# wuxiyang1996/iPLAN

Hardware: AMD Instinct MI355X
Metric: env-steps/sec (whole node), Hetero-Highway chaotic 5-agent (higher is better)
Workload: dtype f32; 1 GPU; Highway chaotic full iPLAN (Behaviour + GAT + soft update), 5 agents x 55 entities, 32 envs/GPU x 90 steps; step = 8 rollouts, each followed by insert + Behavior_policy.learn + Prediction_policy.learn, then IPPOLearner.train (15 epochs x 255 x 90 rows x 5 agents); envs_per_gpu=32

## Files before the change

include/iplan_hip.h:

```cpp
#ifndef IPLAN_HIP_H
#define IPLAN_HIP_H

#include <stddef.h>
#include <stdint.h>

#ifdef __cplusplus
extern "C" {
#endif

typedef void* iplan_stream_t;

enum {
    IPLAN_OK = 0,
    IPLAN_EINVAL = -1,
    IPLAN_EALIGN = -2,
    IPLAN_EHIP = -3
};

const char* iplan_last_error(void);
int iplan_version(void);
size_t iplan_sizeof(const char* struct_name);

#define IPLAN_MAX_ENTITIES 64
#define IPLAN_GAT_HIDDEN 32
// ... 347 lines not shown
    float clip, huber_delta, value_loss_coef;
    float* g_logp;
    float* g_values;
    float* stats;
    const float* mask_sum;
    int32_t flags;
    float row_count;
    int32_t n_parts;
} IplanPpoLossArgs;
#define IPLAN_PPO_MSE 1
#define IPLAN_PPO_NO_VCLIP 2
#define IPLAN_PPO_VALUE_MEAN 4
#define IPLAN_PPO_POLICY_MEAN 8

int iplan_ppo_loss(const IplanPpoLossArgs* args, iplan_stream_t stream);

#define IPLAN_GAT_NODE_DY 640
#define IPLAN_GAT_HARD_PART (8 * IPLAN_GAT_HIDDEN + 16)
#define IPLAN_GAT_WHH_PART (3 * IPLAN_GAT_HIDDEN * IPLAN_GAT_HIDDEN + 3 * IPLAN_GAT_HIDDEN)

typedef struct {
    IplanGatFwdArgs fwd;
    const float* g_out;
    int64_t g_s_net, g_s_b;
    float* dgru;
    float* node_dy;
    float* hard_part;
    float* whh_part;
    float* grad;
    int64_t grad_s_net;
// ... 227 lines not shown
```

iplan_amd/_lib.py:

```python
import ctypes as C
import os

import torch

_HERE = os.path.dirname(os.path.abspath(__file__))
LIB_PATH = os.environ.get("IPLAN_HIP_LIB", os.path.join(_HERE, "libiplan_hip.so"))

GAT_NPARAM = 20
GAT_PARAM_ORDER = [
    "encoding.weight", "encoding.bias",
    "hard_bi_GRU.weight_ih_l0", "hard_bi_GRU.weight_hh_l0", "hard_bi_GRU.bias_ih_l0", "hard_bi_GRU.bias_hh_l0",
    "hard_bi_GRU.weight_ih_l0_reverse", "hard_bi_GRU.weight_hh_l0_reverse",
    "hard_bi_GRU.bias_ih_l0_reverse", "hard_bi_GRU.bias_hh_l0_reverse",
    "hard_encoding.weight", "hard_encoding.bias",
    "q.weight", "k.weight", "v.weight", "v.bias",
    "rnn.weight_ih", "rnn.weight_hh", "rnn.bias_ih", "rnn.bias_hh",
]

fp = C.c_void_p
i32 = C.c_int32
i64 = C.c_int64


class GatSaved(C.Structure):
# ... 8 lines not shown
        ("h_prev", fp), ("h_s_net", i64), ("h_s_b", i64),
        ("out", fp), ("out_s_net", i64), ("out_s_b", i64),
        ("noise", fp), ("params", fp), ("params_s_net", i64),
        ("off", i64 * GAT_NPARAM), ("tau", C.c_float), ("saved", GatSaved), ("phase_clocks", fp),
    ]


class IplanError(RuntimeError):
    pass


ENTRY_POINTS = ["iplan_gat_fwd", "iplan_enc_fwd", "iplan_ac_fwd", "iplan_adam_step", "iplan_wgrad",
                "iplan_ac_bwd_tail", "iplan_ac_bwd_fc1", "iplan_ac_bwd_fc1_finalize", "iplan_ppo_prepare", "iplan_ppo_adv_norm", "iplan_ppo_loss", "iplan_gat_bwd",
                "iplan_pdec_fwd", "iplan_pdec_bwd", "iplan_beh_fwd", "iplan_beh_bwd", "iplan_mlp3_fwd", "iplan_mlp3_bwd", "iplan_seq2seq_fwd", "iplan_ac_pack_fc1",
                "iplan_ac_xhat_pack", "iplan_ac_fc1_split_fwd", "iplan_ac_bwd_fc1_split",
                "iplan_p2p_publish", "iplan_p2p_reduce", "iplan_obs_history_step", "iplan_seq2seq_bwd", "iplan_predict", "iplan_beh_eval"]
RAW_ENTRY_POINTS = ["iplan_grad_sqnorm", "iplan_wgrad_workspace_floats", "iplan_ac_kpad", "iplan_ac_fc1_groups", "iplan_sizeof", "iplan_ac_packed_floats",
                    "iplan_p2p_alloc", "iplan_p2p_free", "iplan_p2p_export", "iplan_p2p_open", "iplan_p2p_close", "iplan_gat_enc_fwd", "iplan_gat_enc_ac_fwd", "iplan_gumbel_noise", "iplan_ac_xhat_floats", "iplan_ac_fc1_split_chunks", "iplan_ac_fc1_split_parts"]


class Lib:

    def __init__(self, cdll):
        self.c = cdll
        cdll.iplan_last_error.restype = C.c_char_p
        cdll.iplan_version.restype = C.c_int
        for name in ENTRY_POINTS:
            if not hasattr(cdll, name):
                raise IplanError(f"{name} missing from the loaded library")
            fn = getattr(cdll, name)
            fn.restype = C.c_int
            fn.argtypes = [C.c_void_p, C.c_void_p]
        for name in RAW_ENTRY_POINTS:
# ... 215 lines not shown

class PpoLossArgs(C.Structure):
    _fields_ = [
        ("n_agents", i32), ("rows", i32), ("row_stride", i64),
        ("logp", fp), ("entropy", fp), ("values", fp), ("old_logp", fp), ("adv", fp),
        ("value_preds", fp), ("returns", fp), ("mask", fp),
        ("clip", C.c_float), ("huber_delta", C.c_float), ("value_loss_coef", C.c_float),
        ("g_logp", fp), ("g_values", fp), ("stats", fp), ("mask_sum", fp), ("flags", i32), ("row_count", C.c_float),
        ("n_parts", i32),
    ]


PPO_MSE, PPO_NO_VCLIP, PPO_VALUE_MEAN, PPO_POLICY_MEAN = 1, 2, 4, 8


GAT_NODE_DY = 640
GAT_HARD_PART = 8 * 32 + 16
GAT_REC_GROUPS = 8
GAT_WHH_PART = 3 * 32 * 32 + 3 * 32


class GatBwdArgs(C.Structure):
    _fields_ = [("fwd", GatFwdArgs), ("g_out", fp), ("g_s_net", i64), ("g_s_b", i64),
                ("dgru", fp), ("node_dy", fp), ("hard_part", fp), ("whh_part", fp), ("grad", fp), ("grad_s_net", i64)]


DEC_PARAM_ORDER = ["decoder.linear.weight", "decoder.linear.bias", "decoder.rnn.weight_ih_l0", "decoder.rnn.weight_hh_l0",
                   "decoder.rnn.bias_ih_l0", "decoder.rnn.bias_hh_l0", "decoder.out.weight", "decoder.out.bias"]
PDEC_SAVE, PDEC_DSAVE = 256, 176

# ... 75 lines not shown
    _fields_ = [("fwd", Seq2SeqArgs), ("g_out", fp), ("dsave", fp)]


class ObsHistArgs(C.Structure):
    _fields_ = [("K", i32), ("nA", i32), ("N", i32), ("L", i32), ("d", i32), ("obs_num", i32),
                ("obs", fp), ("agent_ids", C.c_void_p), ("slot_id", C.c_void_p), ("n_slots", C.c_void_p), ("win", fp), ("single", fp),
                ("single_s_k", i64), ("single_s_a", i64), ("err", C.c_void_p)]


STRUCT_MIRRORS = {"IplanGatSaved": GatSaved, "IplanGatFwdArgs": GatFwdArgs, "IplanGatBwdArgs": GatBwdArgs,
                  "IplanEncFwdArgs": EncFwdArgs, "IplanAcNet": AcNet, "IplanAcFeatures": AcFeatures, "IplanAcFwdArgs": AcFwdArgs,
                  "IplanAcBwdArgs": AcBwdArgs, "IplanAdamArgs": AdamArgs, "IplanWgradProblem": WgradProblem,
                  "IplanWgradArgs": WgradArgs, "IplanPpoPrepareArgs": PpoPrepareArgs, "IplanPpoLossArgs": PpoLossArgs,
                  "IplanPdecArgs": PdecArgs, "IplanBehArgs": BehArgs, "IplanMlp3Args": Mlp3Args, "IplanAdvNormArgs": AdvNormArgs, "IplanSeq2SeqArgs": Seq2SeqArgs, "IplanSeq2SeqBwdArgs": Seq2SeqBwdArgs, "IplanAcPackArgs": AcPackArgs,
                  "IplanIpcHandle": IpcHandle, "IplanP2pArgs": P2pArgs, "IplanAcXhatArgs": AcXhatArgs, "IplanAcFc1SplitArgs": AcFc1SplitArgs,
                  "IplanObsHistArgs": ObsHistArgs, "IplanPredictArgs": PredictArgs, "IplanBehEvalArgs": BehEvalArgs}
```

iplan_amd/csrc/api.cpp:

```cpp
#include <cstring>

#include "api_util.h"

namespace iplan {
char* error_buffer() {
    static thread_local char buf[512] = {0};
    return buf;
}
}

extern "C" const char* iplan_last_error(void) { return iplan::error_buffer(); }
extern "C" int iplan_version(void) { return 100; }

extern "C" size_t iplan_sizeof(const char* name) {
    if (!name) return 0;
#define IPLAN_SZ(T) if (!strcmp(name, #T)) return sizeof(T);
    IPLAN_SZ(IplanGatSaved) IPLAN_SZ(IplanGatFwdArgs) IPLAN_SZ(IplanGatBwdArgs) IPLAN_SZ(IplanEncFwdArgs) IPLAN_SZ(IplanAcNet)
    IPLAN_SZ(IplanAcFeatures) IPLAN_SZ(IplanAcFwdArgs) IPLAN_SZ(IplanAcBwdArgs) IPLAN_SZ(IplanAdamArgs) IPLAN_SZ(IplanWgradProblem)
    IPLAN_SZ(IplanWgradArgs) IPLAN_SZ(IplanPpoPrepareArgs) IPLAN_SZ(IplanPpoLossArgs) IPLAN_SZ(IplanPdecArgs) IPLAN_SZ(IplanBehArgs) IPLAN_SZ(IplanMlp3Args) IPLAN_SZ(IplanAdvNormArgs) IPLAN_SZ(IplanSeq2SeqArgs) IPLAN_SZ(IplanAcPackArgs) IPLAN_SZ(IplanP2pArgs) IPLAN_SZ(IplanIpcHandle) IPLAN_SZ(IplanAcXhatArgs) IPLAN_SZ(IplanAcFc1SplitArgs) IPLAN_SZ(IplanObsHistArgs) IPLAN_SZ(IplanSeq2SeqBwdArgs)
    IPLAN_SZ(IplanPredictArgs) IPLAN_SZ(IplanBehEvalArgs)
#undef IPLAN_SZ
    return 0;
}
```

iplan_amd/learners/ippo_learner.py:

```python
import copy

import os

import torch as th

from .. import _lib as L
from .. import ops
from ..optim import FusedAdam, step_all
from ..streams import AsyncHost
from ..utils.mappo_utils.util import update_linear_schedule

_STORE_KEYS = ("history", "attention_latent", "behavior_latent", "actions", "avail_actions", "reward",
               "terminated", "rnn_states_actors", "rnn_states_critics", "actions_onehot", "obs", "state")


class EpisodeStore:

    def __init__(self, args, device):
        self.size = args.buffer_size
        self.device = device
        self.count = 0
        self.data = {}
        self.consumed = set()

# ... 265 lines not shown
        stats = th.zeros(self.ppo_epoch, nA, parts, 8, **f32)
        norms = th.zeros(self.ppo_epoch, 2, nA, **f32)
        pl.g_logp, pl.g_values = g_logp.data_ptr(), g_v.data_ptr()
        pl.flags = self._loss_flags
        pl.n_parts = parts
        max_norm = self.max_grad_norm if self._use_max_grad_norm else None
        n_rows = float(rows)
        msum = mask[:, :rows].sum(dim=1).contiguous() if (parts > 1 or self.dp is not None) else None
        if self.dp is not None:
            msum = self.dp.all_reduce_sum(msum)
            n_rows = float(self.dp_global_rows if self.dp_global_rows is not None else rows * self.dp.world)
            pl.row_count = n_rows
        if msum is not None:
            pl.mask_sum = msum.data_ptr()
        xhat = ops.ac_xhat_pack(spec, rows, nA, ln_stats) if split else None
        for ep in range(self.ppo_epoch):
            out = ops.ac_forward(mac.actor_arena, mac.critic_arena, 2, spec, rows, nA, save=True, want_entropy=True, xhat=xhat,
                                 packed=None if xhat is not None else mac.fc1_pack.get(spec), **fwd_kw)
            if split and ep == 0:
                old_logp[:, :rows].copy_(out["logp"])
            pl.logp, pl.entropy, pl.values = out["logp"].data_ptr(), out["entropy"].data_ptr(), out["values"].data_ptr()
            pl.stats = stats[ep].data_ptr()
            lib.call("iplan_ppo_loss", pl, stream)
            ops.ac_backward(out, mac.actor_arena, mac.critic_arena, g_logp=g_logp,
                            g_entropy=-self.entropy_coef / n_rows, g_values=g_v)
            if self.dp is not None:
                self.dp.all_reduce_grads(mac.actor_arena, mac.critic_arena)
            self._probe_before(ep, self.ppo_epoch, out)
            sq_a = step_all(self.actor_optimizers, max_norm)
            norms[ep, 0] = sq_a[:, 0]
            sq_c = step_all(self.critic_optimizers, max_norm)
            norms[ep, 1] = sq_c[:, 0]
            self._probe_after(ep)
        self.store.clear()

        st_d = stats.sum(dim=2).mean(dim=(0, 1))
        nr_d = norms.sqrt().mean(dim=(0, 2)) if max_norm is not None else th.zeros(2, device=dev)

        staged = AsyncHost(th.cat([st_d.reshape(-1), nr_d.reshape(-1)])) if defer else None

# ... 300 lines not shown
```

iplan_amd/ops.py:

```python
import contextlib
import ctypes as C

import os

import torch

from . import _lib as L


def _lib(lib):
    return lib if lib is not None else L.get_lib()


def _nb_strides(t, inner):
    assert t.dtype == torch.float32, t.dtype
    expect = 1
    for d in range(t.dim() - 1, 1, -1):
        assert t.stride(d) == expect or t.shape[d] == 1, (t.shape, t.stride())
        expect *= t.shape[d]
    assert expect == inner, (expect, inner)
    return t.stride(0), t.stride(1)


def _gat_flops(n_nets, B, N, D, A, H=32):
# ... 160 lines not shown
        f.T, f.T_phys = self.T, self.T_phys


def _fill_acnet(dst, arena, order, n_out):
    dst.params = arena.data.data_ptr()
    dst.params_s_net = arena.net_stride
    for i, k in enumerate(order):
        dst.off[i] = arena.off(k)
    dst.n_out = n_out


def ac_forward(actor_arena, critic_arena, which, spec, rows, n_agents, h_actor=None, h_critic=None,
               h_strides=(0, 0), avail=None, avail_strides=(0, 0), mode=0, q_noise=None, actions_in=None,
               act_strides=(0, 0), n_actions=5, ksplit=None, save=False, want_probs=False, want_entropy=False,
               want_h=True, h_out=None, actions_out=None, onehot_out=None, ln_stats=None, ln_stats_mode=0, phase_clocks=None,
               packed=None, xhat=None, lib=None, launch=True):
    lib = _lib(lib)
    dev = (actor_arena if which != 1 else critic_arena).data.device
    a = L.AcFwdArgs()
    a.n_agents, a.rows, a.which = n_agents, rows, which
    a.ksplit = ksplit if ksplit is not None else (8 if rows <= 512 else 1)
    a.act_tanh = int(bool(getattr(actor_arena if which != 1 else critic_arena, "act_tanh", False)))
    if which == 2:
        assert bool(getattr(actor_arena, "act_tanh", False)) == bool(getattr(critic_arena, "act_tanh", False)), \
            "actor and critic of one fused launch must use the same trunk activation (args.use_ReLU)"
    spec.fill(a.feat)
    out = {}
    f32 = dict(dtype=torch.float32, device=dev)
    if which != 1:
        _fill_acnet(a.actor, actor_arena, L.ACTOR_PARAM_ORDER, n_actions)
        a.h_actor = h_actor.data_ptr()
# ... 78 lines not shown
        assert which == 2 and a.ksplit == 1 and ln_stats_mode == 2 and xhat["rows"] == rows and xhat["n_agents"] == n_agents
        s = L.AcFc1SplitArgs()
        s.n_agents, s.rows = n_agents, rows
        spec.fill(s.feat)
        s.actor, s.critic = a.actor, a.critic
        KS = (xhat["KT"] + 1) // 2
        ws = workspace(dev, n_agents * KS * 6144 + 2 * n_agents * L.AC_HIDDEN, "fc1_split")
        kparts = int(lib.c.iplan_ac_fc1_split_parts(n_agents, rows))
        z1 = torch.empty(kparts, 2, n_agents, rows, L.AC_HIDDEN, **f32)
        s.kparts, a.fc1_pre_parts = kparts, kparts
        s.xf, s.wsplit, s.wbeta, s.z1 = xhat["xf"].data_ptr(), ws.data_ptr(), ws.data_ptr() + 4 * n_agents * KS * 6144, z1.data_ptr()
        _launch("ac_fc1_split_fwd", lambda: lib.call("iplan_ac_fc1_split_fwd", s, L.current_stream(dev)),
                work=2.0 * n_agents * rows * spec.F * 2 * L.AC_HIDDEN)
        a.fc1_pre = z1.data_ptr()
        out["_xhat"] = xhat
    if launch:
        _launch("ac_fwd_kernel:train" if save else ("ac_fwd_kernel:rollout" if rows <= 512 else "ac_fwd_kernel:infer"),
                lambda: lib.call("iplan_ac_fwd", a, L.current_stream(dev)))
    else:
        assert a.ksplit == 8 and not save and xhat is None and a.ln_stats_mode == 0, "launch=False is for the rollout-shaped forward"
    out["_args"] = a
    out["_keep"] = (spec, h_actor, h_critic, avail, q_noise, actions_in, h_out, actions_out, onehot_out, ln_stats, packed, z1, xhat, ks_bufs)
    return out


def ac_xhat_pack(spec, rows, n_agents, ln_stats, lib=None):
    lib = _lib(lib)
    dev = ln_stats.device
    a = L.AcXhatArgs()
    a.n_agents, a.rows = n_agents, rows
    spec.fill(a.feat)
# ... 230 lines not shown
    w.add(dptr + 4 * M, dst, M, rows, 1, x=sptr + 4 * M, x_strides=sst, K=M,
          dw_off=off("base.mlp.fc2.0.0.weight"), db_off=off("base.mlp.fc2.0.0.bias"))
    w.add(dptr, dst, M, rows, 1, db_off=off("base.mlp.fc1.0.bias"))
    lp = ln_part[which]
    lst = (tiles * 6 * M, 6 * M, 6 * M)
    for k, name in enumerate(("rnn.norm", "base.mlp.fc2.0.2", "base.mlp.fc1.2")):
        w.add(lp.data_ptr() + 4 * (2 * k) * M, lst, M, tiles, 1, db_off=off(name + ".weight"))
        w.add(lp.data_ptr() + 4 * (2 * k + 1) * M, lst, M, tiles, 1, db_off=off(name + ".bias"))
    w._keep += [sv, ds, lp]


def n_which_rows(which, n_agents, rows):
    return (2 if which == 2 else 1) * n_agents * rows


def ac_backward(fwd, actor_arena, critic_arena, g_logp=None, g_entropy=0.0, g_values=None, lib=None):
    lib = _lib(lib)
    fa = fwd["_args"]
    which, n_agents, rows = fa.which, fa.n_agents, fa.rows
    spec, h_actor, h_critic = fwd["_keep"][0], fwd["_keep"][1], fwd["_keep"][2]
    saved = fwd["saved"]
    dev = saved.device
    f32 = dict(dtype=torch.float32, device=dev)
    a = L.AcBwdArgs()
    a.fwd = fa
    if which != 1:
        assert g_logp.shape == (n_agents, rows) and g_logp.is_contiguous()
        a.g_logp = g_logp.data_ptr()
        if torch.is_tensor(g_entropy):
            assert g_entropy.shape == (n_agents, rows) and g_entropy.is_contiguous()
            a.g_entropy = g_entropy.data_ptr()
        else:
            a.g_entropy_const = float(g_entropy)
        a.actor_grad = actor_arena.grad.data_ptr()
        a.actor_grad_s_net = actor_arena.grad.stride(0)
    if which != 0:
        assert g_values.shape == (n_agents, rows) and g_values.is_contiguous()
        a.g_values = g_values.data_ptr()
        a.critic_grad = critic_arena.grad.data_ptr()
        a.critic_grad_s_net = critic_arena.grad.stride(0)
# ... 5 lines not shown
    n_which = 2 if which == 2 else 1
    xhat = fwd.get("_xhat")
    if xhat is not None:
        cr = C.c_int32(0)
        lib.c.iplan_ac_fc1_split_chunks(C.byref(fa.feat), n_agents, rows, C.byref(cr))
        chunk_rows = cr.value
        a.xb = xhat["xb"].data_ptr()
    else:
        k_groups = int(lib.c.iplan_ac_fc1_groups(C.byref(fa.feat)))
        want = max(1, 2048 // (k_groups * n_which * n_agents))
        chunk_rows = max(256, ((rows + want - 1) // want + 15) // 16 * 16)
    chunks = (rows + chunk_rows - 1) // chunk_rows
    g_part = workspace(dev, n_which * n_agents * chunks * L.AC_HIDDEN * Fpad, "fc1")
    a.g_part, a.fc1_chunk_rows, a.fc1_chunks = g_part.data_ptr(), chunk_rows, chunks
    stream = L.current_stream(dev)
    _launch("ac_bwd_tail_kernel", lambda: lib.call("iplan_ac_bwd_tail", a, stream),
            work=4.0 * n_which_rows(which, n_agents, rows) * (8 * L.AC_HIDDEN + 8 + L.AC_HIDDEN + L.AC_DSAVE_FLOATS + L.AC_LNPART_FLOATS / 16.0))
    ev_tail = None
    if which == 2 and dev.type == "cuda":
        ev_tail = torch.cuda.Event()
        ev_tail.record(torch.cuda.current_stream(dev))
    if xhat is not None:
        _launch("ac_fc1_split_wgrad", lambda: lib.call("iplan_ac_bwd_fc1_split", a, stream), work=2.0 * n_agents * rows * spec.F * 2 * L.AC_HIDDEN)
    else:
        lib.call("iplan_ac_bwd_fc1", a, stream)
    T, T_phys = spec.T, spec.T_phys
    hs = (fa.hs_net, fa.hs_row)
    side = None
    if which == 2 and dev.type == "cuda" and not os.environ.get("IPLAN_AC_WGRAD_SERIAL"):
        main = torch.cuda.current_stream(dev)
        side = _side_stream(dev, main.cuda_stream, "ac")
        side.wait_event(ev_tail)
# ... 2 lines not shown
        _ac_wgrad(w, actor_arena, ("act.action_out.linear.weight", "act.action_out.linear.bias"), saved, dsave, 0,
                  n_agents, rows, T, h_actor.data_ptr(), hs, T_phys, fa.actor.n_out, tiles, ln_part)
        w.run(lib)
    if which != 0:
        with (torch.cuda.stream(side) if side is not None else contextlib.nullcontext()):
            w = Wgrad(critic_arena.grad, n_agents)
            _ac_wgrad(w, critic_arena, ("v_out.weight", "v_out.bias"), saved, dsave, 1,
                      n_agents, rows, T, h_critic.data_ptr(), hs, T_phys, 1, tiles, ln_part)
            w.run(lib)
            if side is not None:
                ev_side = torch.cuda.Event()
                ev_side.record(side)
        if side is not None:
            main.wait_event(ev_side)
    lib.call("iplan_ac_bwd_fc1_finalize", a, stream)
    return dict(dsave=dsave, ln_part=ln_part)


def gat_backward(arena, saved, g_out, phase_clocks=None, lib=None):
    lib = _lib(lib)
    fa = saved["_args"]
    src0, src1, h_prev = saved["_keep"][0], saved["_keep"][1], saved["_keep"][2]
    n_nets, B, N, d0, d1 = fa.n_nets, fa.B, fa.N, fa.d0, fa.d1
    H = A = 32
    dev = g_out.device
    f32 = dict(dtype=torch.float32, device=dev)
    a = L.GatBwdArgs()
    a.fwd = fa
    a.g_out = g_out.data_ptr()
    a.g_s_net, a.g_s_b = _nb_strides(g_out, N * A)
    dgru = torch.empty(n_nets, 2, B, (N + 15) // 16, N - 1, 2, 3 * H, **f32)
# ... 527 lines not shown
```

Measured before the change: 89610 env-steps/s.

## Fuse PPO forward tail, loss and backward tail into one-pass kernel

Adds an ac_tail_pass kernel that recomputes the actor/critic forward tail (LN, fc2, GRU cell, head), evaluates the PPO policy and value loss per row, and runs the backward tail in one launch, replacing the separate ac_fwd, ppo_loss and ac_bwd_tail kernels in the full-batch PPO epoch. It also writes only the reduced saved activations unless a probe epoch needs the full record. A small per-agent reduce kernel sums loss statistics from per-workgroup partials. The intent is to cut kernel launches and global-memory round trips of activations and gradients between these stages. The cost is a large LDS-resident weight tile per workgroup, which may limit occupancy, and mask_sum must now be precomputed.

```diff
diff --git a/include/iplan_hip.h b/include/iplan_hip.h
--- a/include/iplan_hip.h
+++ b/include/iplan_hip.h
@@ -385,6 +385,17 @@
 #define IPLAN_PPO_POLICY_MEAN 8
 
 int iplan_ppo_loss(const IplanPpoLossArgs* args, iplan_stream_t stream);
+
+typedef struct {
+    IplanAcBwdArgs bwd;
+    IplanPpoLossArgs loss;
+    float* loss_part;
+    int32_t first_epoch;
+    int32_t full_record;
+    int32_t waves;
+} IplanAcTailPassArgs;
+int iplan_ac_tail_pass_wgs(int32_t rows, int32_t waves);
+int iplan_ac_tail_pass(const IplanAcTailPassArgs* args, iplan_stream_t stream);
 
 #define IPLAN_GAT_NODE_DY 640
 #define IPLAN_GAT_HARD_PART (8 * IPLAN_GAT_HIDDEN + 16)
diff --git a/iplan_amd/_lib.py b/iplan_amd/_lib.py
--- a/iplan_amd/_lib.py
+++ b/iplan_amd/_lib.py
@@ -46,9 +46,11 @@
                 "iplan_ac_bwd_tail", "iplan_ac_bwd_fc1", "iplan_ac_bwd_fc1_finalize", "iplan_ppo_prepare", "iplan_ppo_adv_norm", "iplan_ppo_loss", "iplan_gat_bwd",
                 "iplan_pdec_fwd", "iplan_pdec_bwd", "iplan_beh_fwd", "iplan_beh_bwd", "iplan_mlp3_fwd", "iplan_mlp3_bwd", "iplan_seq2seq_fwd", "iplan_ac_pack_fc1",
                 "iplan_ac_xhat_pack", "iplan_ac_fc1_split_fwd", "iplan_ac_bwd_fc1_split",
-                "iplan_p2p_publish", "iplan_p2p_reduce", "iplan_obs_history_step", "iplan_seq2seq_bwd", "iplan_predict", "iplan_beh_eval"]
+                "iplan_p2p_publish", "iplan_p2p_reduce", "iplan_obs_history_step", "iplan_seq2seq_bwd", "iplan_predict", "iplan_beh_eval",
+                "iplan_ac_tail_pass"]
 RAW_ENTRY_POINTS = ["iplan_grad_sqnorm", "iplan_wgrad_workspace_floats", "iplan_ac_kpad", "iplan_ac_fc1_groups", "iplan_sizeof", "iplan_ac_packed_floats",
-                    "iplan_p2p_alloc", "iplan_p2p_free", "iplan_p2p_export", "iplan_p2p_open", "iplan_p2p_close", "iplan_gat_enc_fwd", "iplan_gat_enc_ac_fwd", "iplan_gumbel_noise", "iplan_ac_xhat_floats", "iplan_ac_fc1_split_chunks", "iplan_ac_fc1_split_parts"]
+                    "iplan_p2p_alloc", "iplan_p2p_free", "iplan_p2p_export", "iplan_p2p_open", "iplan_p2p_close", "iplan_gat_enc_fwd", "iplan_gat_enc_ac_fwd", "iplan_gumbel_noise", "iplan_ac_xhat_floats", "iplan_ac_fc1_split_chunks", "iplan_ac_fc1_split_parts",
+                    "iplan_ac_tail_pass_wgs"]
 
 
 class Lib:
@@ -294,6 +296,10 @@
 PPO_MSE, PPO_NO_VCLIP, PPO_VALUE_MEAN, PPO_POLICY_MEAN = 1, 2, 4, 8
 
 
+class AcTailPassArgs(C.Structure):
+    _fields_ = [("bwd", AcBwdArgs), ("loss", PpoLossArgs), ("loss_part", fp), ("first_epoch", i32), ("full_record", i32), ("waves", i32)]
+
+
 GAT_NODE_DY = 640
 GAT_HARD_PART = 8 * 32 + 16
 GAT_REC_GROUPS = 8
@@ -399,4 +405,5 @@
                   "IplanWgradArgs": WgradArgs, "IplanPpoPrepareArgs": PpoPrepareArgs, "IplanPpoLossArgs": PpoLossArgs,
                   "IplanPdecArgs": PdecArgs, "IplanBehArgs": BehArgs, "IplanMlp3Args": Mlp3Args, "IplanAdvNormArgs": AdvNormArgs, "IplanSeq2SeqArgs": Seq2SeqArgs, "IplanSeq2SeqBwdArgs": Seq2SeqBwdArgs, "IplanAcPackArgs": AcPackArgs,
                   "IplanIpcHandle": IpcHandle, "IplanP2pArgs": P2pArgs, "IplanAcXhatArgs": AcXhatArgs, "IplanAcFc1SplitArgs": AcFc1SplitArgs,
-                  "IplanObsHistArgs": ObsHistArgs, "IplanPredictArgs": PredictArgs, "IplanBehEvalArgs": BehEvalArgs}
+                  "IplanObsHistArgs": ObsHistArgs, "IplanPredictArgs": PredictArgs, "IplanBehEvalArgs": BehEvalArgs,
+                  "IplanAcTailPassArgs": AcTailPassArgs}
diff --git a/iplan_amd/csrc/ac_tail_pass.hip b/iplan_amd/csrc/ac_tail_pass.hip
--- /dev/null
+++ b/iplan_amd/csrc/ac_tail_pass.hip
@@ -0,0 +1,456 @@
+#include "api_util.h"
+#include "gru_tile.h"
+
+namespace iplan {
+
+constexpr int PM = IPLAN_AC_HIDDEN;
+constexpr int PT = PM / 16;
+constexpr int TAIL_PASS_RT = 2;
+constexpr int PLD = PM + 8;
+constexpr int PW_FC2 = 0, PW_WIH = PM, PW_HEAD = 4 * PM, PW_WHH = 4 * PM + 16, PW_ROWS = 7 * PM + 16;
+constexpr int PP_FC1B = 0, PP_LN1W = 64, PP_LN1B = 128, PP_FC2B = 192, PP_LN2W = 256, PP_LN2B = 320, PP_BIH = 384, PP_BHH = 576,
+              PP_LN3W = 768, PP_LN3B = 832, PP_HEADB = 896, PP_FLOATS = 912;
+
+template <int NW>
+struct AcTailPassShared {
+    __attribute__((aligned(16))) float tw[PW_ROWS * PLD];
+    __attribute__((aligned(16))) float tp[PP_FLOATS];
+    float part[NW][4];
+};
+
+__device__ __forceinline__ f32x4 wfrag_lds_t(const float* __restrict__ sW, int ld, int o0, int k0) {
+    const int l = lane_id();
+    const float* p = sW + (k0 + 4 * (l >> 4)) * ld + o0 + (l & 15);
+    f32x4 v;
+    v[0] = p[0]; v[1] = p[ld]; v[2] = p[2 * ld]; v[3] = p[3 * ld];
+    return v;
+}
+
+template <int NA, int KT>
+__device__ __forceinline__ void dense_multi_t(const float* __restrict__ sW, int ld, const int (&o0)[NA], const f32x4* __restrict__ x, f32x4 (&acc)[NA]) {
+    f32x4 f[NA], fn[NA];
+    for (int a = 0; a < NA; ++a) f[a] = wfrag_lds_t(sW, ld, o0[a], 0);
+    for (int T = 0; T < KT; ++T) {
+        if (T + 1 < KT)
+            for (int a = 0; a < NA; ++a) fn[a] = wfrag_lds_t(sW, ld, o0[a], 16 * (T + 1));
+        for (int q = 0; q < 4; ++q)
+            for (int a = 0; a < NA; ++a) acc[a] = mfma4(f[a][q], x[T][q], acc[a]);
+        if (T + 1 < KT)
+            for (int a = 0; a < NA; ++a) f[a] = fn[a];
+    }
+}
+
+__device__ __forceinline__ f32x4 tp_act4(f32x4 v, bool tanh) {
+    f32x4 r;
+    for (int q = 0; q < 4; ++q) r[q] = tanh ? tanh_f(v[q]) : (v[q] > 0.0f ? v[q] : 0.0f);
+    return r;
+}
+
+__device__ __forceinline__ void tp_ln_bwd(f32x4 (&dy)[PT], const f32x4 (&xhat)[PT], const float* __restrict__ gamma, float rstd,
+                                          f32x4 (&dgam)[PT], f32x4 (&dbet)[PT]) {
+    float s1 = 0.f, s2 = 0.f;
+    f32x4 dxh[PT];
+    for (int t = 0; t < PT; ++t) {
+        const f32x4 gm = bfrag_lds(gamma, t);
+        for (int q = 0; q < 4; ++q) {
+            dgam[t][q] = dy[t][q] * xhat[t][q];
+            dbet[t][q] = dy[t][q];
+            dxh[t][q] = dy[t][q] * gm[q];
+            s1 += dxh[t][q];
+            s2 = fmaf(dxh[t][q], xhat[t][q], s2);
+        }
+    }
+    const float m1 = group_sum(s1) * (1.0f / PM), m2 = group_sum(s2) * (1.0f / PM);
+    for (int t = 0; t < PT; ++t)
+        for (int q = 0; q < 4; ++q) dy[t][q] = rstd * (dxh[t][q] - m1 - xhat[t][q] * m2);
+}
+
+__device__ __forceinline__ float tp_chain_sum(float v) {
+    v += __shfl_xor(v, 1);
+    v += __shfl_xor(v, 2);
+    v += __shfl_xor(v, 4);
+    v += __shfl_xor(v, 8);
+    return v;
+}
+
+__device__ __forceinline__ void tp_store_ln_part(float* __restrict__ dst, const f32x4 (&dgam)[PT], const f32x4 (&dbet)[PT]) {
+    const int l = lane_id(), n = l & 15, g = l >> 4;
+    for (int t = 0; t < PT; ++t)
+        for (int q = 0; q < 4; ++q) {
+            const float sg = tp_chain_sum(dgam[t][q]), sb = tp_chain_sum(dbet[t][q]);
+            if (n == 0) {
+                dst[16 * t + 4 * g + q] = sg;
+                dst[PM + 16 * t + 4 * g + q] = sb;
+            }
+        }
+}
+
+__device__ __forceinline__ float tp_huber_q(float e, float d) {
+    const float ae = fabsf(e);
+    return (ae <= d ? e * e * 0.5f : 0.f) + (e > d ? d * (ae - d * 0.5f) : 0.f);
+}
+__device__ __forceinline__ float tp_huber_dq(float e, float d) {
+    return (fabsf(e) <= d ? e : 0.f) + (e > d ? d : 0.f);
+}
+
+template <int NW>
+__global__ __launch_bounds__(64 * NW) void ac_tail_pass_kernel(IplanAcTailPassArgs ta) {
+    __shared__ AcTailPassShared<NW> sh;
+    const IplanAcBwdArgs& a = ta.bwd;
+    const IplanAcFwdArgs& fa = a.fwd;
+    const IplanPpoLossArgs& pl = ta.loss;
+    int bx = (int)blockIdx.x, by = (int)blockIdx.y, bz = (int)blockIdx.z;
+    {
+        const int X = (int)gridDim.x, GY = (int)gridDim.y, G = X * GY * (int)gridDim.z;
+        const int b = bx + X * (by + GY * bz);
+        const int k = b & 7, slot = b >> 3, q8 = G >> 3, r8 = G & 7;
+        const int item = k * q8 + (k < r8 ? k : r8) + slot;
+        bx = item % X;
+        const int pair = item / X;
+        by = pair % GY;
+        bz = pair / GY;
+    }
+    const int net = by, which = bz;
+    const IplanAcNet& nw = which ? fa.critic : fa.actor;
+    const float* __restrict__ P = nw.params + (int64_t)net * nw.params_s_net;
+    const IplanAcFeatures& ft = fa.feat;
+    const int l = lane_id(), w = uniform_i(wave_id()), n = l & 15, g = l >> 4;
+    const bool act_tanh = fa.act_tanh != 0;
+    const bool full = ta.full_record != 0;
+    const int n_out = nw.n_out;
+    {
+        const float* Wsrc[4] = {P + nw.off[IPLAN_AC_FC2_W], P + nw.off[IPLAN_AC_WIH], P + nw.off[IPLAN_AC_HEAD_W], P + nw.off[IPLAN_AC_WHH]};
+        for (int c = (int)threadIdx.x; c < PW_ROWS * 16; c += 64 * NW) {
+            const int r = c >> 4, c4 = c & 15;
+            f32x4 v = splat4(0.f);
+            if (r < PW_WIH) v = *reinterpret_cast<const f32x4*>(Wsrc[0] + r * PM + 4 * c4);
+            else if (r < PW_HEAD) v = *reinterpret_cast<const f32x4*>(Wsrc[1] + (r - PW_WIH) * PM + 4 * c4);
+            else if (r < PW_WHH) { if (r - PW_HEAD < n_out) v = *reinterpret_cast<const f32x4*>(Wsrc[2] + (r - PW_HEAD) * PM + 4 * c4); }
+            else v = *reinterpret_cast<const f32x4*>(Wsrc[3] + (r - PW_WHH) * PM + 4 * c4);
+            *reinterpret_cast<f32x4*>(&sh.tw[r * PLD + 4 * c4]) = v;
+        }
+        const int tp_off[11] = {PP_FC1B, PP_LN1W, PP_LN1B, PP_FC2B, PP_LN2W, PP_LN2B, PP_BIH, PP_BHH, PP_LN3W, PP_LN3B, PP_HEADB};
+        const int tp_src[11] = {IPLAN_AC_FC1_B, IPLAN_AC_LN1_W, IPLAN_AC_LN1_B, IPLAN_AC_FC2_B, IPLAN_AC_LN2_W, IPLAN_AC_LN2_B, IPLAN_AC_BIH,
+                                IPLAN_AC_BHH, IPLAN_AC_LN3_W, IPLAN_AC_LN3_B, IPLAN_AC_HEAD_B};
+#pragma unroll
+        for (int k = 0; k < 11; ++k) {
+            const int len = k == 10 ? 16 : ((k == 6 || k == 7) ? 3 * PM : PM), have = k == 10 ? n_out : len;
+            for (int i = (int)threadIdx.x; i < len; i += 64 * NW) sh.tp[tp_off[k] + i] = i < have ? P[nw.off[tp_src[k]] + i] : 0.f;
+        }
+    }
+    __syncthreads();
+    const float* s_tw = sh.tw;
+    const float* s_tp = sh.tp;
+    const float* sWi = s_tw + PW_WIH * PLD;
+    const float* sWh = s_tw + PW_WHH * PLD;
+    const float* sHd = s_tw + PW_HEAD * PLD;
+    const int tiles = (fa.rows + 15) / 16;
+    const int64_t wrow0 = ((int64_t)which * fa.n_agents + net) * fa.rows;
+    const int o4[PT] = {0, 16, 32, 48};
+    const float msum = pl.mask_sum[net];
+    const float nrow = pl.row_count > 0.f ? pl.row_count : (float)fa.rows;
+    const bool mse = pl.flags & IPLAN_PPO_MSE, no_vclip = pl.flags & IPLAN_PPO_NO_VCLIP;
+    const bool v_mean = pl.flags & IPLAN_PPO_VALUE_MEAN, p_mean = pl.flags & IPLAN_PPO_POLICY_MEAN;
+    const int64_t lo_net = (int64_t)net * pl.row_stride;
+    float pol = 0.f, vls = 0.f, rat = 0.f, en = 0.f;
+
+#pragma unroll 1
+    for (int rt = 0; rt < TAIL_PASS_RT; ++rt) {
+        const int tile = ((bx * NW + w) * TAIL_PASS_RT) + rt;
+        if (tile >= tiles) break;
+        const int r = tile * 16 + n;
+        const bool valid = r < fa.rows;
+        const int rv = valid ? r : 0;
+        const int64_t pr = valid ? (int64_t)(r / ft.T) * ft.T_phys + (r % ft.T) : 0;
+        const int64_t orow = (int64_t)net * fa.rows + rv;
+        float* sv = fa.saved + (wrow0 + rv) * IPLAN_AC_SAVE_FLOATS;
+        float* ds = a.dsave + (wrow0 + rv) * IPLAN_AC_DSAVE_FLOATS;
+        float* lnp = a.ln_part + (((int64_t)which * fa.n_agents + net) * tiles + tile) * IPLAN_AC_LNPART_FLOATS;
+
+        float mu0 = 0.f, rstd0 = 0.f;
+        if (valid) {
+            const float* st = fa.ln_stats + (int64_t)net * fa.ln_stats_s_net + pr * 2;
+            mu0 = st[0]; rstd0 = st[1];
+        }
+        auto load_a1 = [&](f32x4 (&dst)[PT]) {
+            const float* zrow = fa.fc1_pre + (wrow0 + rv) * PM;
+            f32x4 acc[PT];
+            for (int o = 0; o < PT; ++o) acc[o] = vload_a(zrow, valid, o);
+            const int64_t zpart = 2 * (int64_t)fa.n_agents * fa.rows * PM;
+            for (int pp = 1; pp < fa.fc1_pre_parts; ++pp)
+                for (int o = 0; o < PT; ++o) acc[o] += vload_a(zrow + pp * zpart, valid, o);
+            for (int t = 0; t < PT; ++t) dst[t] = tp_act4(acc[t] + bfrag_a(s_tp + PP_FC1B, t), act_tanh);
+        };
+        const float* hsrc = which ? fa.h_critic : fa.h_actor;
+        const float* hrow = hsrc + (int64_t)net * fa.hs_net + pr * fa.hs_row;
+        f32x4 h[PT], hnew[PT], a2[PT], f[PT], f2[PT], gmv[PT], btv[PT];
+        f32x4 gr[PT], gz[PT], gn[PT], ghn[PT];
+        float mu1 = 0.f, rs1 = 0.f, mu2 = 0.f, rs2 = 0.f, mu3 = 0.f, rs3 = 0.f;
+        for (int t = 0; t < PT; ++t) h[t] = vload(hrow, valid, PM, t);
+        load_a1(f);
+        if (full)
+            for (int t = 0; t < PT; ++t) vstore(sv, valid, PM, t, f[t]);
+        for (int t = 0; t < PT; ++t) { gmv[t] = bfrag_a(s_tp + PP_LN1W, t); btv[t] = bfrag_a(s_tp + PP_LN1B, t); }
+        layer_norm_tiles_f<PT>(f, gmv, btv, &mu1, &rs1);
+        for (int t = 0; t < PT; ++t) vstore(sv + PM, valid, PM, t, f[t]);
+        for (int t = 0; t < PT; ++t) {
+            a2[t] = tp_act4(dense_tile<PT>(s_tw, PLD, 16 * t, f, bfrag_a(s_tp + PP_FC2B, t)), act_tanh);
+            f2[t] = a2[t];
+            if (full) vstore(sv + 2 * PM, valid, PM, t, a2[t]);
+        }
+        for (int t = 0; t < PT; ++t) { gmv[t] = bfrag_a(s_tp + PP_LN2W, t); btv[t] = bfrag_a(s_tp + PP_LN2B, t); }
+        layer_norm_tiles_f<PT>(f2, gmv, btv, &mu2, &rs2);
+        for (int t = 0; t < PT; ++t) vstore(sv + 3 * PM, valid, PM, t, f2[t]);
+        for (int t = 0; t < PT; ++t) {
+            f32x4 prr = bfrag_a(s_tp + PP_BIH, t) + bfrag_a(s_tp + PP_BHH, t);
+            f32x4 pz = bfrag_a(s_tp + PP_BIH, PT + t) + bfrag_a(s_tp + PP_BHH, PT + t);
+            f32x4 gni = bfrag_a(s_tp + PP_BIH, 2 * PT + t);
+            f32x4 hn = bfrag_a(s_tp + PP_BHH, 2 * PT + t);
+            prr = dense_tile<PT>(sWh, PLD, 16 * t, h, dense_tile<PT>(sWi, PLD, 16 * t, f2, prr));
+            pz = dense_tile<PT>(sWh, PLD, PM + 16 * t, h, dense_tile<PT>(sWi, PLD, PM + 16 * t, f2, pz));
+            gni = dense_tile<PT>(sWi, PLD, 2 * PM + 16 * t, f2, gni);
+            hn = dense_tile<PT>(sWh, PLD, 2 * PM + 16 * t, h, hn);
+            const GruGates o = gru_gates(prr, pz, gni, hn, h[t]);
+            IPLAN_SCHED_FENCE();
+            hnew[t] = o.h;
+            gr[t] = o.r; gz[t] = o.z; gn[t] = o.n; ghn[t] = o.hn;
+            if (full) {
+                vstore(sv + 4 * PM, valid, PM, t, o.r);
+                vstore(sv + 5 * PM, valid, PM, t, o.z);
+                vstore(sv + 6 * PM, valid, PM, t, o.n);
+                vstore(sv + 7 * PM, valid, PM, t, o.hn);
+                vstore(sv + 8 * PM, valid, PM, t, o.h);
+            }
+        }
+        float* hout = which ? fa.h_critic_out : fa.h_actor_out;
+        if (hout) {
+            float* horow = fa.ho_s_row ? hout + (int64_t)net * fa.ho_s_net + (int64_t)rv * fa.ho_s_row : hout + ((int64_t)net * fa.rows + rv) * PM;
+            for (int t = 0; t < PT; ++t) vstore(horow, valid, PM, t, hnew[t]);
+        }
+        f32x4 f3[PT];
+        for (int t = 0; t < PT; ++t) f3[t] = hnew[t];
+        for (int t = 0; t < PT; ++t) { gmv[t] = bfrag_a(s_tp + PP_LN3W, t); btv[t] = bfrag_a(s_tp + PP_LN3B, t); }
+        layer_norm_tiles_f<PT>(f3, gmv, btv, &mu3, &rs3);
+        for (int t = 0; t < PT; ++t) vstore(sv + 9 * PM, valid, PM, t, f3[t]);
+        if (valid && g == 0) {
+            float* st = sv + 10 * PM;
+            st[0] = mu0; st[1] = rstd0; st[2] = mu1; st[3] = rs1; st[4] = mu2; st[5] = rs2; st[6] = mu3; st[7] = rs3;
+        }
+        const f32x4 lg = dense_tile<PT>(sHd, PLD, 0, f3, bfrag_a(s_tp + PP_HEADB, 0));
+
+        IPLAN_SCHED_FENCE();
+        f32x4 dhead[1];
+        dhead[0] = splat4(0.f);
+        if (which == 1) {
+            const float v = lg[0];
+            if (valid && g == 0) {
+                if (fa.values) fa.values[orow] = v;
+                const float m = pl.mask[lo_net + r];
+                const float wv = v_mean ? 1.0f / nrow : m / msum;
+                const float vp = pl.value_preds[lo_net + r], rtn = pl.returns[lo_net + r];
+                const float dv = v - vp;
+                const float vc = vp + fminf(fmaxf(dv, -pl.clip), pl.clip);
+                const float e1 = rtn - v, e2 = rtn - vc;
+                const float h1 = mse ? 0.5f * e1 * e1 : tp_huber_q(e1, pl.huber_delta), h2 = mse ? 0.5f * e2 * e2 : tp_huber_q(e2, pl.huber_delta);
+                const float d1 = -(mse ? e1 : tp_huber_dq(e1, pl.huber_delta));
+                const float d2 = (dv >= -pl.clip && dv <= pl.clip) ? -(mse ? e2 : tp_huber_dq(e2, pl.huber_delta)) : 0.f;
+                vls += (no_vclip ? h1 : fmaxf(h1, h2)) * wv;
+                const float dvl = (no_vclip || h1 > h2) ? d1 : (h2 > h1 ? d2 : 0.5f * (d1 + d2));
+                const float gv = pl.value_loss_coef * wv * dvl;
+                if (pl.g_values) pl.g_values[orow] = gv;
+                dhead[0][0] = gv;
+            }
+        } else {
+            f32x4 x;
+            bool masked[4];
+            float m = -INFINITY;
+            for (int q = 0; q < 4; ++q) {
+                const int idx = 4 * g + q;
+                x[q] = lg[q];
+                masked[q] = false;
+                if (idx < n_out) {
+                    if (fa.avail && valid && fa.avail[(int64_t)net * fa.av_s_net + pr * fa.av_s_row + idx] == 0) { x[q] = -1e10f; masked[q] = true; }
+                    m = fmaxf(m, x[q]);
+                }
+            }
+            m = fmaxf(m, __shfl_xor(m, 16));
+            m = fmaxf(m, __shfl_xor(m, 32));
+            f32x4 e;
+            float se = 0.f;
+            for (int q = 0; q < 4; ++q) { e[q] = (4 * g + q < n_out) ? expf(x[q] - m) : 0.f; se += e[q]; }
+            se = group_sum(se);
+            const float lse = m + logf(se);
+            f32x4 lp, pb;
+            for (int q = 0; q < 4; ++q) { lp[q] = x[q] - lse; pb[q] = e[q] / se; }
+            const int action = valid ? (int)fa.actions_in[(int64_t)net * fa.act_s_net + pr * fa.act_s_row] : 0;
+            float sel = 0.f, ent = 0.f;
+            for (int q = 0; q < 4; ++q) {
+                const int idx = 4 * g + q;
+                if (idx < n_out) {
+                    if (idx == action) sel += lp[q];
+                    ent -= pb[q] * lp[q];
+                    if (fa.probs && valid) fa.probs[orow * n_out + idx] = pb[q];
+                }
+            }
+            sel = group_sum(sel);
+            ent = group_sum(ent);
+            float glp = 0.f;
+            if (valid) {
+                const float mk = pl.mask[lo_net + r], ad = pl.adv[lo_net + r];
+                const float old_lp = ta.first_epoch ? sel : pl.old_logp[lo_net + r];
+                const float ratio = expf(sel - old_lp);
+                const float lo = 1.0f - pl.clip, hi = 1.0f + pl.clip;
+                const float rc = fminf(fmaxf(ratio, lo), hi);
+                const float s1 = ratio * ad, s2 = rc * ad;
+                const float wp = p_mean ? 1.0f / nrow : mk / msum;
+                const bool inside = ratio >= lo && ratio <= hi;
+                float dr = 0.f;
+                if (s1 < s2) dr = ad;
+                else if (s1 == s2) dr = inside ? ad : 0.5f * ad;
+                glp = -wp * dr * ratio;
+                if (g == 0) {
+                    pol -= fminf(s1, s2) * wp;
+                    rat += ratio;
+                    en += ent;
+                    if (fa.logp) fa.logp[orow] = sel;
+                    if (fa.entropy) fa.entropy[orow] = ent;
+                    if (pl.g_logp) pl.g_logp[orow] = glp;
+                }
+            }
+            const float gen = valid ? (a.g_entropy ? a.g_entropy[orow] : a.g_entropy_const) : 0.f;
+            for (int q = 0; q < 4; ++q) {
+                const int idx = 4 * g + q;
+                float d = 0.f;
+                if (idx < n_out && !masked[q]) {
+                    d = glp * ((idx == action ? 1.0f : 0.0f) - pb[q]);
+                    d -= gen * pb[q] * (lp[q] + ent);
+                }
+                dhead[0][q] = d;
+            }
+        }
+        vstore(ds + 6 * PM, valid, 16, 0, dhead[0]);
+
+        IPLAN_SCHED_FENCE();
+        f32x4 dgam[PT], dbet[PT];
+        f32x4 d[PT];
+        for (int t = 0; t < PT; ++t) d[t] = splat4(0.f);
+        dense_multi_t<PT, 1>(sHd, PLD, o4, dhead, d);
+        {
+            f32x4 xh[PT];
+            for (int t = 0; t < PT; ++t)
+                for (int q = 0; q < 4; ++q) xh[t][q] = (hnew[t][q] - mu3) * rs3;
+            tp_ln_bwd(d, xh, s_tp + PP_LN3W, rs3, dgam, dbet);
+            tp_store_ln_part(lnp, dgam, dbet);
+        }
+        IPLAN_SCHED_FENCE();
+        f32x4 dg[3 * PT];
+        for (int t = 0; t < PT; ++t) {
+            const GruGrads o = gru_gates_bwd(d[t], gr[t], gz[t], gn[t], ghn[t], vload(hrow, valid, PM, t));
+            dg[t] = o.dr;
+            dg[PT + t] = o.dz;
+            dg[2 * PT + t] = o.dni;
+            vstore(ds + 2 * PM, valid, PM, t, o.dr);
+            vstore(ds + 3 * PM, valid, PM, t, o.dz);
+            vstore(ds + 4 * PM, valid, PM, t, o.dni);
+            vstore(ds + 5 * PM, valid, PM, t, o.dnh);
+        }
+        IPLAN_SCHED_FENCE();
+        for (int t = 0; t < PT; ++t) d[t] = splat4(0.f);
+        dense_multi_t<PT, 3 * PT>(sWi, PLD, o4, dg, d);
+        {
+            f32x4 xh[PT];
+            for (int t = 0; t < PT; ++t)
+                for (int q = 0; q < 4; ++q) xh[t][q] = (a2[t][q] - mu2) * rs2;
+            tp_ln_bwd(d, xh, s_tp + PP_LN2W, rs2, dgam, dbet);
+            tp_store_ln_part(lnp + 2 * PM, dgam, dbet);
+            for (int t = 0; t < PT; ++t) {
+                for (int q = 0; q < 4; ++q) d[t][q] = act_tanh ? d[t][q] * (1.0f - a2[t][q] * a2[t][q]) : (a2[t][q] > 0.f ? d[t][q] : 0.f);
+                vstore(ds + PM, valid, PM, t, d[t]);
+            }
+        }
+        {
+            f32x4 df1[PT];
+            for (int t = 0; t < PT; ++t) df1[t] = splat4(0.f);
+            dense_multi_t<PT, PT>(s_tw, PLD, o4, d, df1);
+            for (int t = 0; t < PT; ++t) d[t] = df1[t];
+        }
+        {
+            f32x4 xh[PT], a1[PT];
+            load_a1(a1);
+            for (int t = 0; t < PT; ++t)
+                for (int q = 0; q < 4; ++q) xh[t][q] = (a1[t][q] - mu1) * rs1;
+            tp_ln_bwd(d, xh, s_tp + PP_LN1W, rs1, dgam, dbet);
+            tp_store_ln_part(lnp + 4 * PM, dgam, dbet);
+            for (int t = 0; t < PT; ++t) {
+                for (int q = 0; q < 4; ++q) d[t][q] = act_tanh ? d[t][q] * (1.0f - a1[t][q] * a1[t][q]) : (a1[t][q] > 0.f ? d[t][q] : 0.f);
+                vstore(ds, valid, PM, t, d[t]);
+            }
+        }
+    }
+
+    pol = wave_sum(pol);
+    vls = wave_sum(vls);
+    rat = wave_sum(rat);
+    en = wave_sum(en);
+    if (l == 0) { sh.part[w][0] = pol; sh.part[w][1] = vls; sh.part[w][2] = rat; sh.part[w][3] = en; }
+    __syncthreads();
+    if (threadIdx.x < 4) {
+        float s = 0.f;
+        for (int k = 0; k < NW; ++k) s += sh.part[k][threadIdx.x];
+        ta.loss_part[((((int64_t)which * fa.n_agents + net) * (int64_t)gridDim.x) + bx) * 4 + threadIdx.x] = s;
+    }
+}
+
+__global__ __launch_bounds__(64) void ac_tail_loss_reduce_kernel(IplanAcTailPassArgs ta, int wgs) {
+    const int net = (int)blockIdx.x, k = (int)threadIdx.x;
+    const IplanPpoLossArgs& pl = ta.loss;
+    const int n_agents = ta.bwd.fwd.n_agents;
+    if (k >= 4) return;
+    const int which = k == 1 ? 1 : 0;
+    const float* p = ta.loss_part + ((int64_t)which * n_agents + net) * wgs * 4 + k;
+    float s = 0.f;
+    for (int i = 0; i < wgs; ++i) s += p[4 * i];
+    const int P = pl.n_parts > 1 ? pl.n_parts : 1;
+    float* st = pl.stats + (int64_t)net * P * 8;
+    const float n = (float)ta.bwd.fwd.rows;
+    st[k] = k >= 2 ? s / n : s;
+    if (k == 0) st[4] = pl.mask_sum[net];
+}
+
+}
+
+static int tail_pass_waves(int waves) { return waves == 16 ? 16 : 8; }
+
+extern "C" int iplan_ac_tail_pass_wgs(int rows, int waves) {
+    const int tiles = (rows + 15) / 16;
+    const int per = tail_pass_waves(waves) * iplan::TAIL_PASS_RT;
+    return (tiles + per - 1) / per;
+}
+
+extern "C" int iplan_ac_tail_pass(const IplanAcTailPassArgs* ta, iplan_stream_t stream) {
+    using namespace iplan;
+    if (!ta) return fail(IPLAN_EINVAL, "iplan_ac_tail_pass: null args");
+    const IplanAcBwdArgs& a = ta->bwd;
+    const IplanAcFwdArgs& f = a.fwd;
+    const IplanPpoLossArgs& pl = ta->loss;
+    if (f.which != 2 || f.n_agents < 1 || f.rows < 1 || f.mode != 2 || f.ksplit != 1 || !f.actions_in || !f.h_actor || !f.h_critic)
+        return fail(IPLAN_EINVAL, "iplan_ac_tail_pass: needs both nets (which 2), mode 2 with actions_in, ksplit 1 and the stored hidden states");
+    if (!f.fc1_pre || !aligned16(f.fc1_pre) || f.ln_stats_mode != 2 || !f.ln_stats)
+        return fail(IPLAN_EINVAL, "iplan_ac_tail_pass: needs fc1_pre and stored LayerNorm statistics (ln_stats_mode 2)");
+    if (f.feat.T < 1 || f.feat.T_phys < f.feat.T) return fail(IPLAN_EINVAL, "iplan_ac_tail_pass: bad T/T_phys");
+    if (f.actor.n_out < 1 || f.actor.n_out > 16) return fail(IPLAN_EINVAL, "iplan_ac_tail_pass: n_actions=%d outside [1,16]", f.actor.n_out);
+    if (!f.saved || !a.dsave || !a.ln_part || !ta->loss_part)
+        return fail(IPLAN_EINVAL, "iplan_ac_tail_pass: saved / dsave / ln_part / loss_part missing");
+    if (pl.n_agents != f.n_agents || pl.rows != f.rows || pl.row_stride < f.rows || !pl.adv || !pl.value_preds || !pl.returns || !pl.mask ||
+        !pl.mask_sum || !pl.stats || (!ta->first_epoch && !pl.old_logp))
+        return fail(IPLAN_EINVAL, "iplan_ac_tail_pass: bad loss arguments (mask_sum is required: the gradients' denominator is fixed before the launch)");
+    if (ta->waves != 0 && ta->waves != 8 && ta->waves != 16) return fail(IPLAN_EINVAL, "iplan_ac_tail_pass: waves must be 0, 8 or 16");
+    const int waves = tail_pass_waves(ta->waves);
+    const int wgs = iplan_ac_tail_pass_wgs(f.rows, waves);
+    dim3 grid((unsigned)wgs, (unsigned)f.n_agents, 2u);
+    if (waves == 16) hipLaunchKernelGGL((ac_tail_pass_kernel<16>), grid, dim3(1024), 0, (hipStream_t)stream, *ta);
+    else hipLaunchKernelGGL((ac_tail_pass_kernel<8>), grid, dim3(512), 0, (hipStream_t)stream, *ta);
+    if (int rc = check_launch("iplan_ac_tail_pass")) return rc;
+    hipLaunchKernelGGL(ac_tail_loss_reduce_kernel, dim3((unsigned)f.n_agents), dim3(64), 0, (hipStream_t)stream, *ta, wgs);
+    return check_launch("iplan_ac_tail_pass (loss reduce)");
+}
diff --git a/iplan_amd/csrc/api.cpp b/iplan_amd/csrc/api.cpp
--- a/iplan_amd/csrc/api.cpp
+++ b/iplan_amd/csrc/api.cpp
@@ -18,7 +18,7 @@
     IPLAN_SZ(IplanGatSaved) IPLAN_SZ(IplanGatFwdArgs) IPLAN_SZ(IplanGatBwdArgs) IPLAN_SZ(IplanEncFwdArgs) IPLAN_SZ(IplanAcNet)
     IPLAN_SZ(IplanAcFeatures) IPLAN_SZ(IplanAcFwdArgs) IPLAN_SZ(IplanAcBwdArgs) IPLAN_SZ(IplanAdamArgs) IPLAN_SZ(IplanWgradProblem)
     IPLAN_SZ(IplanWgradArgs) IPLAN_SZ(IplanPpoPrepareArgs) IPLAN_SZ(IplanPpoLossArgs) IPLAN_SZ(IplanPdecArgs) IPLAN_SZ(IplanBehArgs) IPLAN_SZ(IplanMlp3Args) IPLAN_SZ(IplanAdvNormArgs) IPLAN_SZ(IplanSeq2SeqArgs) IPLAN_SZ(IplanAcPackArgs) IPLAN_SZ(IplanP2pArgs) IPLAN_SZ(IplanIpcHandle) IPLAN_SZ(IplanAcXhatArgs) IPLAN_SZ(IplanAcFc1SplitArgs) IPLAN_SZ(IplanObsHistArgs) IPLAN_SZ(IplanSeq2SeqBwdArgs)
-    IPLAN_SZ(IplanPredictArgs) IPLAN_SZ(IplanBehEvalArgs)
+    IPLAN_SZ(IplanPredictArgs) IPLAN_SZ(IplanBehEvalArgs) IPLAN_SZ(IplanAcTailPassArgs)
 #undef IPLAN_SZ
     return 0;
 }
diff --git a/iplan_amd/learners/ippo_learner.py b/iplan_amd/learners/ippo_learner.py
--- a/iplan_amd/learners/ippo_learner.py
+++ b/iplan_amd/learners/ippo_learner.py
@@ -303,16 +303,27 @@
         if msum is not None:
             pl.mask_sum = msum.data_ptr()
         xhat = ops.ac_xhat_pack(spec, rows, nA, ln_stats) if split else None
+        one_pass = split and os.environ.get("IPLAN_PPO_TAIL", "fused") != "split"
+        if one_pass and msum is None:
+            msum = mask[:, :rows].sum(dim=1).contiguous()
+            pl.mask_sum = msum.data_ptr()
         for ep in range(self.ppo_epoch):
             out = ops.ac_forward(mac.actor_arena, mac.critic_arena, 2, spec, rows, nA, save=True, want_entropy=True, xhat=xhat,
-                                 packed=None if xhat is not None else mac.fc1_pack.get(spec), **fwd_kw)
-            if split and ep == 0:
-                old_logp[:, :rows].copy_(out["logp"])
-            pl.logp, pl.entropy, pl.values = out["logp"].data_ptr(), out["entropy"].data_ptr(), out["values"].data_ptr()
+                                 packed=None if xhat is not None else mac.fc1_pack.get(spec), tail=not one_pass, **fwd_kw)
             pl.stats = stats[ep].data_ptr()
-            lib.call("iplan_ppo_loss", pl, stream)
-            ops.ac_backward(out, mac.actor_arena, mac.critic_arena, g_logp=g_logp,
-                            g_entropy=-self.entropy_coef / n_rows, g_values=g_v)
+            if one_pass:
+                probe = (self.probe_last_step and ep == self.ppo_epoch - 1) or ep in self.probe_steps
+                ops.ac_backward(out, mac.actor_arena, mac.critic_arena, g_logp=g_logp, g_entropy=-self.entropy_coef / n_rows, g_values=g_v, loss=pl,
+                                first_epoch=ep == 0, full_record=probe)
+                if ep == 0:
+                    old_logp[:, :rows].copy_(out["logp"])
+            else:
+                if split and ep == 0:
+                    old_logp[:, :rows].copy_(out["logp"])
+                pl.logp, pl.entropy, pl.values = out["logp"].data_ptr(), out["entropy"].data_ptr(), out["values"].data_ptr()
+                lib.call("iplan_ppo_loss", pl, stream)
+                ops.ac_backward(out, mac.actor_arena, mac.critic_arena, g_logp=g_logp,
+                                g_entropy=-self.entropy_coef / n_rows, g_values=g_v)
             if self.dp is not None:
                 self.dp.all_reduce_grads(mac.actor_arena, mac.critic_arena)
             self._probe_before(ep, self.ppo_epoch, out)
diff --git a/iplan_amd/ops.py b/iplan_amd/ops.py
--- a/iplan_amd/ops.py
+++ b/iplan_amd/ops.py
@@ -198,7 +198,7 @@
                h_strides=(0, 0), avail=None, avail_strides=(0, 0), mode=0, q_noise=None, actions_in=None,
                act_strides=(0, 0), n_actions=5, ksplit=None, save=False, want_probs=False, want_entropy=False,
                want_h=True, h_out=None, actions_out=None, onehot_out=None, ln_stats=None, ln_stats_mode=0, phase_clocks=None,
-               packed=None, xhat=None, lib=None, launch=True):
+               packed=None, xhat=None, lib=None, launch=True, tail=True):
     lib = _lib(lib)
     dev = (actor_arena if which != 1 else critic_arena).data.device
     a = L.AcFwdArgs()
@@ -307,7 +307,9 @@
                 work=2.0 * n_agents * rows * spec.F * 2 * L.AC_HIDDEN)
         a.fc1_pre = z1.data_ptr()
         out["_xhat"] = xhat
-    if launch:
+    if not tail:
+        assert xhat is not None and save and mode == 2, "tail=False is for the full-batch PPO epoch (xhat, save, mode 2)"
+    elif launch:
         _launch("ac_fwd_kernel:train" if save else ("ac_fwd_kernel:rollout" if rows <= 512 else "ac_fwd_kernel:infer"),
                 lambda: lib.call("iplan_ac_fwd", a, L.current_stream(dev)))
     else:
@@ -568,7 +570,8 @@
     return (2 if which == 2 else 1) * n_agents * rows
 
 
-def ac_backward(fwd, actor_arena, critic_arena, g_logp=None, g_entropy=0.0, g_values=None, lib=None):
+def ac_backward(fwd, actor_arena, critic_arena, g_logp=None, g_entropy=0.0, g_values=None, lib=None, loss=None,
+                first_epoch=False, full_record=False):
     lib = _lib(lib)
     fa = fwd["_args"]
     which, n_agents, rows = fa.which, fa.n_agents, fa.rows
@@ -578,6 +581,10 @@
     f32 = dict(dtype=torch.float32, device=dev)
     a = L.AcBwdArgs()
     a.fwd = fa
+    if loss is not None:
+        assert which == 2 and fwd.get("_xhat") is not None, "the one-pass tail is the full-batch (xhat) route of both nets"
+        g_logp = torch.empty(n_agents, rows, **f32) if g_logp is None else g_logp
+        g_values = torch.empty(n_agents, rows, **f32) if g_values is None else g_values
     if which != 1:
         assert g_logp.shape == (n_agents, rows) and g_logp.is_contiguous()
         a.g_logp = g_logp.data_ptr()
@@ -613,8 +620,20 @@
     g_part = workspace(dev, n_which * n_agents * chunks * L.AC_HIDDEN * Fpad, "fc1")
     a.g_part, a.fc1_chunk_rows, a.fc1_chunks = g_part.data_ptr(), chunk_rows, chunks
     stream = L.current_stream(dev)
-    _launch("ac_bwd_tail_kernel", lambda: lib.call("iplan_ac_bwd_tail", a, stream),
-            work=4.0 * n_which_rows(which, n_agents, rows) * (8 * L.AC_HIDDEN + 8 + L.AC_HIDDEN + L.AC_DSAVE_FLOATS + L.AC_LNPART_FLOATS / 16.0))
+    loss_part = None
+    if loss is not None:
+        t = L.AcTailPassArgs()
+        t.bwd, t.loss = a, loss
+        t.first_epoch, t.full_record = int(bool(first_epoch)), int(bool(full_record))
+        t.waves = int(os.environ.get("IPLAN_PPO_TAIL_WAVES", "0"))
+        t.loss.g_logp, t.loss.g_values = g_logp.data_ptr(), g_values.data_ptr()
+        loss_part = torch.empty(2, n_agents, int(lib.c.iplan_ac_tail_pass_wgs(rows, t.waves)), 4, **f32)
+        t.loss_part = loss_part.data_ptr()
+        _launch("ac_tail_pass_kernel", lambda: lib.call("iplan_ac_tail_pass", t, stream),
+                work=4.0 * n_which_rows(which, n_agents, rows) * (2 * L.AC_HIDDEN + 3 * L.AC_HIDDEN + 8 + L.AC_DSAVE_FLOATS + L.AC_LNPART_FLOATS / 16.0))
+    else:
+        _launch("ac_bwd_tail_kernel", lambda: lib.call("iplan_ac_bwd_tail", a, stream),
+                work=4.0 * n_which_rows(which, n_agents, rows) * (8 * L.AC_HIDDEN + 8 + L.AC_HIDDEN + L.AC_DSAVE_FLOATS + L.AC_LNPART_FLOATS / 16.0))
     ev_tail = None
     if which == 2 and dev.type == "cuda":
         ev_tail = torch.cuda.Event()
@@ -647,7 +666,7 @@
         if side is not None:
             main.wait_event(ev_side)
     lib.call("iplan_ac_bwd_fc1_finalize", a, stream)
-    return dict(dsave=dsave, ln_part=ln_part)
+    return dict(dsave=dsave, ln_part=ln_part, loss_part=loss_part)
 
 
 def gat_backward(arena, saved, g_out, phase_clocks=None, lib=None):
```

Result: no change. 90610 env-steps/s, median of 6 (+1.1%).
